# LemonATsu/DANBO-pytorch

Measured on AMD Instinct MI355X. Metric: ray-samples/sec at 512x512x64 samples, higher is better.
Workload: dtype f32 (fp16x2-split MFMA products, fp32 accumulate); 1 GPU; H36M danbo_base network, 512x512 rays x (48 coarse + 16 importance) samples, 1 pose / 1 camera per rank, cylinder near/far, exact in-volume culling; rays=262144, samples_per_ray=64, parallelism=rays-dp1

## Files before the change

danbo-pytorch_amd/core/render_engine.py:

```python
import ctypes

import torch

from . import _hip
from . import hip_ops as ops


class RenderEngine:
    fuse_resample = False

    def _key(self):
        return tuple((k, v.data_ptr(), v._version) for k, v in sorted(self.p.items()))

    def _sampling(self, N_samples, N_importance):
        cfg = self.cfg
        return (N_samples or cfg["N_samples"], N_importance or cfg["N_importance"], cfg["density_scale"],
                ops.density_act(cfg.get("density_act")))

    @staticmethod
    def frame_result(out, out0):
        return dict(rgb_map=out["rgb_map"], disp_map=out["disp_map"], acc_map=out["acc_map"], alpha=out["alpha"],
                    T_i=out["weights"], rgb0=out0["rgb_map"], disp0=out0["disp_map"], acc0=out0["acc_map"],
                    alpha0=out0["alpha"])

# ... 20 lines not shown
        ret = self.frame_result(out, out0)
        if keep:
            ret.update(near=near, far=far, z_coarse=z, raw_coarse=raw, weights_coarse=out0["weights"], z_fine=z_fine,
                       z_sorted=z_all, sorted_idxs=order, raw_fine=raw_f, **ex, **ex_f)
        return ret


class DanboEngine(RenderEngine):
    fuse_resample = True

    def __init__(self, cfg, params, align, buffers=None, mlp_mode="f16split"):
        self.cfg = cfg
        self.p = params
        self.align = align.float().contiguous()
        self._packed_key = None
        self.packed = self.wrt = self.empty_consts = None
        self.mean_code = None
        self.profile = None
        self.skip_flat_rays = True
        self.mlp_form = 32
        assert mlp_mode in ("f16split", "fp32")
        self.mlp_mode = mlp_mode
        self.group_rows = False

    def refresh(self):
        key = self._key()
        if key == self._packed_key and getattr(self, "_built_mode", None) == (self.mlp_mode, self.mlp_form):
            return
        p = self.p
        dev = p["alpha_linear.weight"].device
        q = self._equalized(p) if self.mlp_mode == "f16split" else p
        self.pts_w = [q[f"pts_linears.{i}.weight"] for i in range(8)]
        self.pts_b = [q[f"pts_linears.{i}.bias"].contiguous() for i in range(8)]
        self.packed, self.wrt = ops.mlp_pack(self.pts_w, q["feature_linear.weight"], q["views_linears.0.weight"])
        self.packed16, self.views_b16 = ops.mlp16_pack(self.pts_w, q["feature_linear.weight"],
                                                       q["feature_linear.bias"], q["views_linears.0.weight"],
                                                       q["views_linears.0.bias"], form=self.mlp_form)
        self.alpha_w = q["alpha_linear.weight"].reshape(-1).contiguous()
        self.alpha_b = q["alpha_linear.bias"].contiguous()
        self.feature_b = q["feature_linear.bias"].contiguous()
        self.views_b = q["views_linears.0.bias"].contiguous()
        self.rgb_w = q["rgb_linear.weight"].contiguous()
        self.rgb_b = q["rgb_linear.bias"].contiguous()
        self.view_scale = q.get("_view_scale", torch.ones((), device=dev))
        g = "graph_net.layers."
        self.gw = dict(
# ... 198 lines not shown
        o = _hip.DanboFrameOut(**{k: v.data_ptr() for k, v in out.items()})
        nbytes = _hip.lib().danbo_render_frame_workspace(R, G, S, Sf, int(chunk), m.graph_width)
        ws = torch.empty(nbytes, device=dev, dtype=torch.uint8)
        ops._call("danbo_render_frame_act", ctypes.byref(m), ctypes.byref(r), S, Sf, ctypes.byref(o), _hip.ptr(ws), nbytes,
                  *ops._act_args(act), ops._stream())
        out["T_i"] = out.pop("weights")
        return out

    def near_far(self, rays_o, rays_d, cyls, skts, near0=0.0, far0=1.0, chunk=4096):
        self.refresh()
        near, far = ops.near_far_cylinder(rays_o, rays_d, cyls, near0, far0, chunk)
        if self.cfg["use_volume_near_far"]:
            ops.near_far_boxes(rays_o, rays_d, skts, self.align, self.axis_scale, near, far)
        return near, far

    def render(self, rays_o, rays_d, skts, bones, cyls, cam_idx=None, N_samples=None, N_importance=None,
               chunk=4096, near_far=None, dense=False, keep=False):
        S, Sf, B, act = self._sampling(N_samples, N_importance)
        self.refresh()
        fused = S <= 64 and Sf <= 64
        lazy = not dense and not keep
        flat_mode = (lazy and (fused or (S <= 256 and Sf <= 64)) and self.skip_flat_rays and self.flat_rays_ok
                     and act[0] == "relu")
        near, far = self.near_far(rays_o, rays_d, cyls, skts, 0.0, 1.0, chunk) if near_far is None else near_far
        z = ops.coarse_samples(near, far, S)
        ray_mask = None if dense else ops.ray_bone_mask(rays_o, rays_d, skts, self.align, self.axis_scale, near, far,
                                                        want_flat=flat_mode)
        counts = torch.zeros(3, device=rays_o.device, dtype=torch.int32)
        flat = None
        vols = self.volumes(bones)
        if flat_mode:
            flat = ops.flat_rays(ray_mask[1], ray_mask[3], S, Sf, want_weights=not fused, cnt=counts[2:3])
            view = self.view_constants(rays_d, skts, cam_idx, flat["ray_list"], flat["ray_count"])
        else:
            view = self.view_constants(rays_d, skts, cam_idx)
        if ray_mask is not None:
            ray_mask = ray_mask[:3]
        raw, ex = self.forward_samples(rays_o, rays_d, skts, bones, cam_idx, z=z, dense=dense, volumes=vols, view=view,
                                       fill=not lazy, ray_mask=ray_mask, count=counts[0:1])
        if fused:
            out0, z_all, z_fine, order = ops.composite_importance(
                raw, z, rays_d, Sf, B, bits=ex["valid_bits"] if lazy else None, raw_empty=view[1] if lazy else None,
                want_weights=keep, flat=flat, act=act)
        else:
            out0 = ops.composite(raw, z, rays_d, B, bits=ex["valid_bits"] if lazy else None, raw_empty=view[1] if lazy else None,
                                 flat=flat, act=act)
# ... 22 lines not shown
```

danbo-pytorch_amd/csrc/k_frame.hip:

```cpp
#include "common.hpp"

using namespace danbo;

namespace {
struct Carver {
    char* base;
    size_t used, cap;
    template <class T>
    T* take(size_t n) {
        used = (used + 255) & ~(size_t)255;
        T* p = base ? reinterpret_cast<T*>(base + used) : nullptr;
        used += n * sizeof(T);
        return p;
    }
};

struct FrameBuffers {
    float *near, *far, *cyl_scratch, *z, *vol_scratch, *volumes, *cview, *raw_empty, *h, *raw_a, *raw_b, *z_fine, *z_sorted, *weights0;
    uint32_t *bits_a, *bits_b, *ray_mask, *ray_flat;
    int32_t *list, *count, *order, *ray_list;
};

FrameBuffers carve(Carver& c, int R, int G, int S, int Sf, int chunk, int Wg) {
    FrameBuffers b;
    const size_t M = (size_t)R * S, Mf = (size_t)R * Sf;
    b.near = c.take<float>(R);
    b.far = c.take<float>(R);
    b.cyl_scratch = c.take<float>(8 * (size_t)((R + chunk - 1) / chunk));
    b.z = c.take<float>(M);
    b.vol_scratch = c.take<float>(3 * (size_t)G * 24 * Wg);
    b.volumes = c.take<float>((size_t)G * 24 * 240);
    b.cview = c.take<float>((size_t)R * 128);
    b.raw_empty = c.take<float>((size_t)R * 4);
    b.ray_mask = c.take<uint32_t>(R);
    b.ray_flat = c.take<uint32_t>(R);
    b.ray_list = c.take<int32_t>(R);
    b.bits_a = c.take<uint32_t>(M);
    b.bits_b = c.take<uint32_t>(Mf);
    b.list = c.take<int32_t>(M);
    b.count = c.take<int32_t>(4);
    b.h = c.take<float>((M > Mf ? M : Mf) * 16);
    b.raw_a = c.take<float>(M * 4);
    b.raw_b = c.take<float>(Mf * 4);
    b.z_fine = c.take<float>(Mf);
    b.z_sorted = c.take<float>(M + Mf);
    b.order = c.take<int32_t>(M + Mf);
    if (Mf > M) b.list = c.take<int32_t>(Mf);
    b.weights0 = (S <= 64 && Sf <= 64) ? nullptr : c.take<float>(M);
    return b;
}
}

extern "C" size_t danbo_render_frame_workspace(int R, int G, int S, int Sf, int chunk, int graph_width) {
    if (R < 1 || G < 1 || S < 1 || Sf < 1 || chunk < 1 || graph_width < 1) return 0;
    Carver c{nullptr, 0, 0};
    carve(c, R, G, S, Sf, chunk, graph_width);
    return c.used + 256;
}

#define DANBO_TRY(call) do { const int rc_ = (call); if (rc_ != 0) return rc_; } while (0)

static int render_frame_impl(const DanboModel* m, const DanboRays* r, int S, int Sf, const DanboFrameOut* o, void* workspace,
                             size_t workspace_bytes, int act, float shift, void* stream) {
    DANBO_CHECK_ARG(m && r && o && workspace && S >= 3 && S <= 256 && Sf >= 1 && Sf <= 64);
    DANBO_CHECK_ARG(r->R >= 1 && r->G >= 1 && r->R % r->G == 0 && r->chunk >= 1);
    DANBO_CHECK_ARG(r->rays_o && r->rays_d && r->skts && r->bones && r->cyls);
    DANBO_CHECK_ARG(o->rgb_map && o->disp_map && o->acc_map && o->alpha && o->weights && o->rgb0 && o->disp0 && o->acc0 && o->alpha0);
    const int R = r->R, G = r->G;
    const bool flat_rays = m->flat_rays_ok != 0 && act == DANBO_DENSITY_RELU;
    DANBO_CHECK_ARG(workspace_bytes >= danbo_render_frame_workspace(R, G, S, Sf, r->chunk, m->graph_width));
    Carver c{reinterpret_cast<char*>(((uintptr_t)workspace + 255) & ~(uintptr_t)255), 0, workspace_bytes};
    const FrameBuffers b = carve(c, R, G, S, Sf, r->chunk, m->graph_width);
    hipStream_t st = (hipStream_t)stream;

    DANBO_TRY(danbo_near_far_cylinder(r->rays_o, r->rays_d, r->cyls, R, G, 0.f, 1.f, r->near_in, r->far_in, r->chunk, b.cyl_scratch,
                                      b.near, b.far, stream));
    if (m->use_volume_near_far)
        DANBO_TRY(danbo_near_far_boxes(r->rays_o, r->rays_d, r->skts, m->align, m->axis_scale, R, G, b.near, b.far, stream));
    DANBO_TRY(danbo_coarse_samples(b.near, b.far, R, S, nullptr, b.z, stream));
    DANBO_TRY(danbo_ray_bone_mask(r->rays_o, r->rays_d, b.near, b.far, R, G, r->skts, m->align, m->axis_scale, b.ray_mask,
                                  flat_rays ? b.ray_flat : nullptr, stream));
    DANBO_TRY(danbo_pose_volumes_fwd(r->bones, G, m->L_graph, m->graph_width, m->g_w0, m->g_adjw0, m->g_b0, m->g_w1, m->g_adjw1, m->g_b1,
                                     m->g_w2, m->g_b2, m->g_w3, m->g_b3, b.vol_scratch, b.volumes, stream));
    zero_words(b.count, 4, nullptr, 0, st);
    auto view_consts = [&](const int32_t* ray_list, const int32_t* ray_count) -> int {
        return danbo_view_consts(r->rays_d, r->skts, R, G, m->ray_mode, m->normalise, m->L_view, m->framecodes, m->n_codes, m->code_size,
                                 m->mean_code, r->cam_idx, m->views_w_ray_t, m->views_b_eff, m->rgb_w, m->rgb_b, m->empty_consts, 2,
                                 m->code_table, ray_list, ray_count, b.cview, b.raw_empty, stream);
    };
    const int32_t *ray_list = nullptr, *ray_count = nullptr;
    if (flat_rays) {
        DANBO_TRY(danbo_flat_rays(b.near, b.ray_flat, R, S, Sf, o->rgb0, o->disp0, o->acc0, b.weights0, o->alpha0, b.z_fine, o->rgb_map,
                                  o->disp_map, o->acc_map, o->weights, o->alpha, b.ray_list, b.count + 3, 3, stream));
        ray_list = b.ray_list;
        ray_count = b.count + 3;
    }
    DANBO_TRY(view_consts(ray_list, ray_count));
    auto cull = [&](const float* zz, int s, uint32_t* bits, int32_t* count) -> int {
        DANBO_TRY(danbo_bone_cull(r->rays_o, r->rays_d, zz, nullptr, R, s, G, r->skts, m->align, m->axis_scale, b.ray_mask, b.near, b.far,
                                  nullptr, bits, b.list, count, stream));
        return 0;
    };
    auto network = [&](const float* zz, int s, uint32_t* bits, int32_t* count, float* raw) -> int {
        DANBO_TRY(danbo_gather_assign_blend16_fwd(r->rays_o, r->rays_d, zz, nullptr, R, s, G, r->skts, m->align, m->axis_scale, b.volumes,
                                                  bits, b.list, count, R * s, m->assign16, m->a_b0, m->a_b1, m->a_w2, m->a_b2, b.h,
                                                  nullptr, reinterpret_cast<uint32_t*>(b.count + 2), stream));
        return danbo_pe_mlp32_fwd(b.h, b.list, count, R * s, s, m->mlp16, m->pts_b, m->alpha_w, m->alpha_b, b.cview, m->rgb_w,
                                  m->rgb_b, raw, nullptr, stream);
    };
    DANBO_TRY(cull(b.z, S, b.bits_a, b.count));
    DANBO_TRY(network(b.z, S, b.bits_a, b.count, b.raw_a));
    if (S <= 64) {
        DANBO_TRY(danbo_composite_importance_pdf_fwd_act(b.raw_a, b.raw_empty, b.bits_a, b.z, r->rays_d, R, S, Sf, m->density_scale, nullptr,
                                                         nullptr, 0, o->rgb0, o->disp0, o->acc0, nullptr, o->alpha0, b.z_fine, b.z_sorted,
                                                         b.order, ray_list, ray_count, act, shift, stream));
    } else {
        DANBO_TRY(danbo_composite_rays_fwd_act(b.raw_a, b.raw_empty, b.bits_a, b.z, r->rays_d, R, S, m->density_scale, nullptr, o->rgb0,
                                               o->disp0, o->acc0, b.weights0, o->alpha0, ray_list, ray_count, act, shift, stream));
        DANBO_TRY(danbo_importance_samples_rays(b.z, b.weights0, R, S, Sf, nullptr, b.z_fine, b.z_sorted, b.order, ray_list, ray_count,
                                                stream));
    }
    DANBO_TRY(cull(b.z_fine, Sf, b.bits_b, b.count + 1));
    DANBO_TRY(network(b.z_fine, Sf, b.bits_b, b.count + 1, b.raw_b));
// ... 16 lines not shown
```

danbo-pytorch_amd/csrc/k_sample.hip:

```cpp
#include "common.hpp"

namespace danbo {

__global__ __launch_bounds__(256) DANBO_NO_PK_F32 void k_cylinder_pass1(const float* __restrict__ rays_o,
                                                        const float* __restrict__ rays_d,
                                                        const float* __restrict__ cyl, int R, int G,
                                                        float near0, float far0,
                                                        const float* __restrict__ near_in,
                                                        const float* __restrict__ far_in, int chunk,
                                                        double* __restrict__ acc,
                                                        float* __restrict__ near_out,
                                                        float* __restrict__ far_out) {
    const int rays_per_pose = R / G;
    for (int r0 = blockIdx.x * blockDim.x; r0 < R; r0 += gridDim.x * blockDim.x) {
        const int r = r0 + threadIdx.x;
        const bool act = r < R;
        const int rc = act ? r : R - 1;
        const int g = min(rc / rays_per_pose, G - 1);
        float o[3] = {rays_o[3 * rc], rays_o[3 * rc + 1], rays_o[3 * rc + 2]};
        float d[3] = {rays_d[3 * rc], rays_d[3 * rc + 1], rays_d[3 * rc + 2]};
        float c[3] = {cyl[5 * g], cyl[5 * g + 1], cyl[5 * g + 2]};
        float nr, fr;
        const bool hit = cylinder_bounds(o, d, c, near_in ? near_in[rc] : near0, far_in ? far_in[rc] : far0, &nr, &fr) && act;
        if (act) {
// ... 241 lines not shown
    bone_local(sk, al, o, ol);
    for (int k = 0; k < 3; ++k) t[k] = sk[4 * k] * d[0] + sk[4 * k + 1] * d[1] + sk[4 * k + 2] * d[2];
    for (int k = 0; k < 3; ++k) dl[k] = al[4 * k] * t[0] + al[4 * k + 1] * t[1] + al[4 * k + 2] * t[2];
    const float pad = 1e-4f * fmaxf(fabsf(zl), fabsf(zh)) + 1e-5f;
    float tmin = zl - pad, tmax = zh + pad;
    bool miss = false;
    for (int k = 0; k < 3; ++k) {
        const float s = sc[k] * 1.001f + 1e-4f;
        if (fabsf(dl[k]) < 1e-12f) {
            miss = miss || fabsf(ol[k]) > s;
        } else {
            const float inv = 1.0f / dl[k];
            const float t1 = (-s - ol[k]) * inv, t2 = (s - ol[k]) * inv;
            tmin = fmaxf(tmin, fminf(t1, t2));
            tmax = fminf(tmax, fmaxf(t1, t2));
        }
    }
    return miss || tmin > tmax;
}

constexpr float RAY_FLAT_VMAX = DANBO_RAY_FLAT_VMAX;

template <bool POSES_IN_LDS>
__global__ __launch_bounds__(256) void k_ray_bone_mask(const float* __restrict__ rays_o, const float* __restrict__ rays_d,
                                                       const float* __restrict__ t_lo, const float* __restrict__ t_hi,
                                                       const float* __restrict__ skts, const float* __restrict__ align,
                                                       const float* __restrict__ axis_scale, int R, int G,
                                                       uint32_t* __restrict__ ray_mask, uint32_t* __restrict__ ray_flat) {
    extern __shared__ __attribute__((aligned(16))) float smem[];
    float* s_align = smem;
    float* s_scale = smem + J * 16;
    float* s_skt = smem + J * 16 + J * 4;
    const int rays_per_pose = R / G;
    const int r_a = blockIdx.x * 256, r_b = min(r_a + 255, R - 1);
    const int g0 = min(r_a / rays_per_pose, G - 1), g1 = min(r_b / rays_per_pose, G - 1);
    const int r = min(r_a + (int)threadIdx.x, R - 1);
    const float o[3] = {rays_o[3 * r], rays_o[3 * r + 1], rays_o[3 * r + 2]};
    const float d[3] = {rays_d[3 * r], rays_d[3 * r + 1], rays_d[3 * r + 2]};
    const float zl = t_lo[r], zh = t_hi[r];
    for (int i = threadIdx.x; i < J * 16; i += 256) s_align[i] = align[i];
    for (int i = threadIdx.x; i < J * 4; i += 256) s_scale[i] = (i & 3) < 3 ? fabsf(axis_scale[(i >> 2) * 3 + (i & 3)]) : 0.f;
    if (POSES_IN_LDS)
        for (int i = threadIdx.x; i < (g1 - g0 + 1) * J * 16; i += 256) s_skt[i] = skts[(size_t)g0 * J * 16 + i];
    __syncthreads();
    const int g = min(r / rays_per_pose, G - 1);
    uint32_t bits = 0u;
    if (POSES_IN_LDS) {
        const float* sk = s_skt + (size_t)(g - g0) * J * 16;
#pragma unroll 2
        for (int j = 0; j < J; ++j)
            bits |= segment_misses_bone(sk + 16 * j, s_align + 16 * j, s_scale + 4 * j, o, d, zl, zh) ? 0u : 1u << j;
    } else {
        for (int j = 0; j < J; ++j) {
            float sk[12];
            const float* src = skts + ((size_t)g * J + j) * 16;
#pragma unroll
            for (int i = 0; i < 12; ++i) sk[i] = src[i];
            bits |= segment_misses_bone(sk, s_align + 16 * j, s_scale + 4 * j, o, d, zl, zh) ? 0u : 1u << j;
        }
    }
    if (r_a + (int)threadIdx.x < R) {
        ray_mask[r] = bits;
        if (ray_flat != nullptr) {
            const float dn = norm3_torch(d[0], d[1], d[2]);
            const float span = mul_rn(add_rn(sub_rn(zh, zl), mul_rn(1e-3f, fmaxf(fabsf(zl), fabsf(zh)))), dn);
            const float tail = mul_rn(1e10f, dn);
            const float* m0 = POSES_IN_LDS ? s_skt + (size_t)(g - g0) * J * 16 : skts + (size_t)g * J * 16;
            float msum = 0.f;
            for (int a = 0; a < 3; ++a)
                for (int k = 0; k < 3; ++k) msum = add_rn(msum, fabsf(m0[4 * a + k]));
            const float vin = mul_rn(dn, fmaxf(1.0f, msum));
            const bool fin = zl <= zh && sub_rn(span, span) == 0.f && sub_rn(tail, tail) == 0.f && vin <= RAY_FLAT_VMAX;
            ray_flat[r] = (bits == 0u && fin) ? 1u : 0u;
        }
    }
}

constexpr int CULL_BLOCK = 256;
constexpr int CULL_SPT = 4;
constexpr int CULL_MAX_RAYS = 130;

__global__ __launch_bounds__(CULL_BLOCK) void k_bone_cull(const float* __restrict__ rays_o,
                                                          const float* __restrict__ rays_d,
                                                          const float* __restrict__ z,
                                                          const float* __restrict__ pts, int R, int S, int G,
                                                          const float* __restrict__ skts,
                                                          const float* __restrict__ align,
                                                          const float* __restrict__ axis_scale, int np_lds,
                                                          const uint32_t* __restrict__ ray_mask,
                                                          const float* __restrict__ t_lo, const float* __restrict__ t_hi,
                                                          uint32_t* __restrict__ ray_flat,
                                                          uint32_t* __restrict__ valid_bits,
                                                          int32_t* __restrict__ list, int32_t* __restrict__ count) {
    extern __shared__ __attribute__((aligned(16))) float smem[];
    float* s_align = smem;
    float* s_scale = smem + J * 16;
    float* s_skt = smem + J * 16 + J * 4;
    __shared__ float s_zlo[CULL_MAX_RAYS], s_zhi[CULL_MAX_RAYS];
    __shared__ uint32_t s_mask[CULL_MAX_RAYS];

    const long M = (long)R * S;
    const long spp = (long)(R / G) * S;
    const long base = (long)blockIdx.x * (CULL_BLOCK * CULL_SPT);
// ... 92 lines not shown
        const int lia = (int)(mac - base) + off0, lib = (int)(mbc - base) + off0;
        const int ra = r_first + ray_of(lia), rb = r_first + ray_of(lib);
        float pa[3], pb[3];
        if (pts != nullptr) {
            pa[0] = pts[3 * mac]; pa[1] = pts[3 * mac + 1]; pa[2] = pts[3 * mac + 2];
            pb[0] = pts[3 * mbc]; pb[1] = pts[3 * mbc + 1]; pb[2] = pts[3 * mbc + 2];
        } else {
            const float oa[3] = {rays_o[3 * ra], rays_o[3 * ra + 1], rays_o[3 * ra + 2]};
            const float da[3] = {rays_d[3 * ra], rays_d[3 * ra + 1], rays_d[3 * ra + 2]};
            const float ob[3] = {rays_o[3 * rb], rays_o[3 * rb + 1], rays_o[3 * rb + 2]};
            const float db[3] = {rays_d[3 * rb], rays_d[3 * rb + 1], rays_d[3 * rb + 2]};
            sample_point(oa, da, ma < M ? zreg[2 * pr] : z[M - 1], pa);
            sample_point(ob, db, mb < M ? zreg[2 * pr + 1] : z[M - 1], pb);
        }
        const int ga = pose_of(ra), gb = pose_of(rb);
        uint32_t ba = 0, bb = 0;
        uint32_t need = (1u << J) - 1u;
        if (ray_mask != nullptr) {
            need = wave_or(pre[2 * pr] | pre[2 * pr + 1]);
        } else if (prefilter) {
            uint32_t mine = s_mask[ra - r_first] | s_mask[rb - r_first];
            need = wave_or(mine);
        }
        if (__builtin_amdgcn_readfirstlane((int)__all(ga == gb))) {
            const v2f px = {pa[0], pb[0]}, py = {pa[1], pb[1]}, pz = {pa[2], pb[2]};
            const float* sk = s_skt + (ga - g0) * J * 16;
            while (need) {
                const int j = __builtin_ctz(need);
                need &= need - 1u;
                v2f l[3], t[3];
                affine_pk(sk + 16 * j, px, py, pz, l);
                affine_pk(s_align + 16 * j, l[0], l[1], l[2], t);
                const float* sc = s_scale + 4 * j;
                const bool ina = !(fabsf(t[0].x) > sc[0] || fabsf(t[1].x) > sc[1] || fabsf(t[2].x) > sc[2]);
                const bool inb = !(fabsf(t[0].y) > sc[0] || fabsf(t[1].y) > sc[1] || fabsf(t[2].y) > sc[2]);
                ba |= (ina ? 1u : 0u) << j;
                bb |= (inb ? 1u : 0u) << j;
            }
        } else {
            const float* ska = s_skt + (ga - g0) * J * 16;
            const float* skb = s_skt + (gb - g0) * J * 16;
            for (int j = 0; j < J; ++j) {
                float pt[3];
                bone_local(ska + 16 * j, s_align + 16 * j, pa, pt);
                ba |= (in_volume(pt, s_scale + 4 * j) ? 1u : 0u) << j;
                bone_local(skb + 16 * j, s_align + 16 * j, pb, pt);
                bb |= (in_volume(pt, s_scale + 4 * j) ? 1u : 0u) << j;
            }
        }
        bits4[2 * pr] = ma < M ? ba : 0u;
        bits4[2 * pr + 1] = mb < M ? bb : 0u;
        if (ma < M) valid_bits[ma] = ba;
        if (mb < M) valid_bits[mb] = bb;
    }
    if (list != nullptr) {
        __shared__ int s_cnt[CULL_SPT * (CULL_BLOCK / 64)];
        __shared__ int s_base;
        const int wave = threadIdx.x >> 6;
        unsigned long long ball[CULL_SPT];
#pragma unroll
        for (int it = 0; it < CULL_SPT; ++it) {
            ball[it] = __ballot(bits4[it] != 0);
            if (lane == 0) s_cnt[it * (CULL_BLOCK / 64) + wave] = __popcll(ball[it]);
        }
        __syncthreads();
        if (threadIdx.x == 0) {
            int run = 0;
            for (int i = 0; i < CULL_SPT * (CULL_BLOCK / 64); ++i) { const int c = s_cnt[i]; s_cnt[i] = run; run += c; }
            s_base = run > 0 ? atomicAdd(count, run) : 0;
        }
        __syncthreads();
#pragma unroll
        for (int it = 0; it < CULL_SPT; ++it) {
            if (bits4[it] != 0) {
                const long m = base + it * CULL_BLOCK + threadIdx.x;
                list[s_base + s_cnt[it * (CULL_BLOCK / 64) + wave] + __popcll(ball[it] & ((1ull << lane) - 1ull))] = (int32_t)m;
            }
        }
    }
}

constexpr int GATHER_TS = 16;
constexpr int GATHER_BLOCK = GATHER_TS * J;

__global__ __launch_bounds__(GATHER_BLOCK) void k_bone_gather(const float* __restrict__ rays_o,
                                                              const float* __restrict__ rays_d,
                                                              const float* __restrict__ z,
                                                              const float* __restrict__ pts, int R, int S, int G,
                                                              const float* __restrict__ skts,
                                                              const float* __restrict__ align,
                                                              const float* __restrict__ axis_scale,
                                                              const float* __restrict__ volumes,
                                                              const int32_t* __restrict__ list,
                                                              const int32_t* __restrict__ count, int n_cap,
                                                              float* __restrict__ part_feat) {
    __shared__ __attribute__((aligned(16))) float s_vol[J * VOL];
    __shared__ __attribute__((aligned(16))) float s_out[GATHER_TS * J * FEAT];
    __shared__ __attribute__((aligned(16))) float s_skt[J * 16];
    __shared__ __attribute__((aligned(16))) float s_align[J * 16];
    __shared__ float s_scale[J * 4];

    const int n = resolve_count(count, n_cap);
// ... 528 lines not shown
        for (int c = lane; c < S; c += 64) {
            if (weights0) weights0[rr * S + c] = 0.f;
            if (alpha0) alpha0[rr * S + c] = 0.f;
        }
        const float lo_b = __builtin_bit_cast(float, __builtin_amdgcn_readlane(__builtin_bit_cast(int, lo), b));
        for (int c = lane; c < Sf; c += 64) z_fine[rr * Sf + c] = lo_b;
        for (int c = lane; c < St; c += 64) {
            if (weights) weights[rr * St + c] = 0.f;
            if (alpha_out) alpha_out[rr * St + c] = 0.f;
        }
    }
    if (!(parts & 1)) return;
    if (lane == 0) s_cnt[wave] = (int)__popcll(listed);
    __syncthreads();
    if (threadIdx.x == 0) {
        int run = 0;
        for (int w = 0; w < FLAT_BLOCK / 64; ++w) { const int c = s_cnt[w]; s_cnt[w] = run; run += c; }
        s_base = run > 0 ? atomicAdd(ray_count, run) : 0;
    }
    __syncthreads();
    if (r < R && !flat) ray_list[s_base + s_cnt[wave] + (int)__popcll(listed & ((1ull << lane) - 1ull))] = r;
}

}

using namespace danbo;

static unsigned ray_scatter(int R) {
    static const unsigned primes[] = {40507u, 40519u, 40529u, 40531u, 40543u, 40559u};
    for (unsigned p : primes) {
        unsigned a = p, b = (unsigned)R;
        while (b != 0u) { const unsigned t = a % b; a = b; b = t; }
        if (a == 1u) return p;
    }
    return 1u;
}

extern "C" int danbo_near_far_cylinder(const float* rays_o, const float* rays_d, const float* cyl, int R, int G,
                                        float near0, float far0, const float* near_in, const float* far_in, int chunk,
                                        float* scratch, float* near_out, float* far_out, void* stream) {
    DANBO_CHECK_ARG(R > 0 && G > 0 && R % G == 0 && chunk > 0 && scratch != nullptr);
    hipStream_t st = (hipStream_t)stream;
    const int nchunk = ceil_div(R, chunk);
    if (chunk <= CYL_FUSED_MAX) {
        hipLaunchKernelGGL(k_cylinder_chunk, dim3(nchunk), dim3(CYL_BLOCK), 0, st, rays_o, rays_d, cyl, R, G, near0, far0, near_in,
                           far_in, chunk, near_out, far_out);
// ... 28 lines not shown
                           far, R, S, t_rand, z);
    DANBO_LAUNCH_RET();
}

extern "C" int danbo_bone_cull(const float* rays_o, const float* rays_d, const float* z, const float* pts, int R, int S, int G,
                                const float* skts, const float* align, const float* axis_scale, const uint32_t* ray_mask,
                                const float* t_lo, const float* t_hi, uint32_t* ray_flat, uint32_t* valid_bits, int32_t* list,
                                int32_t* count, void* stream) {
    DANBO_CHECK_ARG(R > 0 && S > 0 && G > 0 && R % G == 0);
    DANBO_CHECK_ARG((list == nullptr) == (count == nullptr));
    DANBO_CHECK_ARG((z == nullptr) != (pts == nullptr));
    DANBO_CHECK_ARG(ray_mask == nullptr || (z != nullptr && t_lo != nullptr && t_hi != nullptr));
    DANBO_CHECK_ARG(ray_flat == nullptr || ray_mask != nullptr);
    const long M = (long)R * S;
    const long spp = (long)(R / G) * S;
    const int per_block = CULL_BLOCK * CULL_SPT;
    long np = per_block / spp + 2;
    if (np > G) np = G;
    const size_t lds = sizeof(float) * (J * 16 + J * 4 + np * J * 16);
    DANBO_CHECK_ARG(lds <= 64 * 1024);
    const int grid = ceil_div(M, per_block);
    hipLaunchKernelGGL(k_bone_cull, dim3(grid), dim3(CULL_BLOCK), lds, (hipStream_t)stream, rays_o, rays_d, z, pts, R, S,
                       G, skts, align, axis_scale, (int)np, ray_mask, t_lo, t_hi, ray_flat, valid_bits, list, count);
    DANBO_LAUNCH_RET();
}

extern "C" int danbo_ray_bone_mask(const float* rays_o, const float* rays_d, const float* t_lo, const float* t_hi, int R, int G,
                                    const float* skts, const float* align, const float* axis_scale, uint32_t* ray_mask,
                                    uint32_t* ray_flat, void* stream) {
    DANBO_CHECK_ARG(rays_o && rays_d && t_lo && t_hi && skts && align && axis_scale && ray_mask);
    DANBO_CHECK_ARG(R > 0 && G > 0 && R % G == 0);
    const long np = 256 / (R / G) + 2 < G ? 256 / (R / G) + 2 : G;
    const bool in_lds = np <= 8;
    const size_t lds = sizeof(float) * (J * 16 + J * 4 + (in_lds ? np * J * 16 : 0));
    if (in_lds)
        hipLaunchKernelGGL(k_ray_bone_mask<true>, dim3(ceil_div(R, 256)), dim3(256), lds, (hipStream_t)stream, rays_o, rays_d, t_lo, t_hi,
                           skts, align, axis_scale, R, G, ray_mask, ray_flat);
    else
        hipLaunchKernelGGL(k_ray_bone_mask<false>, dim3(ceil_div(R, 256)), dim3(256), lds, (hipStream_t)stream, rays_o, rays_d, t_lo,
                           t_hi, skts, align, axis_scale, R, G, ray_mask, ray_flat);
    DANBO_LAUNCH_RET();
}

extern "C" int danbo_bone_gather_fwd(const float* rays_o, const float* rays_d, const float* z, const float* pts, int R, int S, int G,
                                      const float* skts, const float* align, const float* axis_scale,
                                      const float* volumes, const int32_t* list, const int32_t* count, int n,
// ... 157 lines not shown
                                                       int act, float shift, void* stream) {
    DANBO_CHECK_ARG(pdf == 0 || pdf == 1);
    DANBO_CHECK_DENSITY_ACT(act, shift);
#define DANBO_CI(TWO_, DA_, SH_)                                                                                                   \
    composite_importance_impl<TWO_, DA_>(raw, raw_empty, valid_bits, z, rays_d, R, S, Sf, B, noise, u, rgb_map, disp, acc, weights, \
                                         alpha, z_fine, z_sorted, sorted_idx, ray_list, ray_count, SH_, stream)
    if (act == DENSITY_SOFTPLUS) return pdf ? DANBO_CI(true, DENSITY_SOFTPLUS, shift) : DANBO_CI(false, DENSITY_SOFTPLUS, shift);
    return pdf ? DANBO_CI(true, DENSITY_RELU, 0.f) : DANBO_CI(false, DENSITY_RELU, 0.f);
#undef DANBO_CI
}

extern "C" int danbo_flat_rays(const float* t_lo, const uint32_t* ray_flat, int R, int S, int Sf, float* rgb0, float* disp0, float* acc0, float* weights0, float* alpha0, float* z_fine,
                                float* rgb_map, float* disp, float* acc, float* weights, float* alpha, int32_t* ray_list,
                                int32_t* ray_count, int parts, void* stream) {
    DANBO_CHECK_ARG(R > 0 && S >= 3 && Sf > 0);
    DANBO_CHECK_ARG(t_lo && ray_flat && rgb0 && disp0 && acc0 && z_fine && rgb_map && disp && acc && ray_list && ray_count);
    DANBO_CHECK_ARG(parts >= 1 && parts <= 3);
    hipLaunchKernelGGL(k_flat_rays, dim3(ceil_div(R, FLAT_BLOCK)), dim3(FLAT_BLOCK), 0, (hipStream_t)stream,
                       t_lo, ray_flat, R, S, Sf, rgb0, disp0, acc0, weights0, alpha0, z_fine,
                       rgb_map, disp, acc, weights, alpha, ray_list, ray_count, parts);
    DANBO_LAUNCH_RET();
}

template <int DA>
static int composite_merged_impl(const float* raw_a, const float* raw_b, const float* raw_empty,
                                 const uint32_t* bits_a, const uint32_t* bits_b, const int32_t* sorted_idx,
                                 const float* z_sorted, const float* rays_d, int R, int S, int Sf, float B,
                                 const float* noise, float* rgb_map, float* disp, float* acc, float* weights,
                                 float* alpha, float* raw_sorted, const int32_t* ray_list, const int32_t* ray_count,
                                 float shift, void* stream) {
    DANBO_CHECK_ARG(R > 0 && S > 0 && Sf > 0 && B > 0.f && raw_a && raw_b && sorted_idx && z_sorted && rays_d);
    DANBO_CHECK_ARG(rgb_map && disp && acc && ((bits_a == nullptr && bits_b == nullptr) || raw_empty != nullptr));
    DANBO_CHECK_ARG((ray_list == nullptr) == (ray_count == nullptr));
    const float4 *a4 = reinterpret_cast<const float4*>(raw_a), *b4 = reinterpret_cast<const float4*>(raw_b);
    const float4* e4 = reinterpret_cast<const float4*>(raw_empty);
    float4* rs4 = reinterpret_cast<float4*>(raw_sorted);
    if constexpr (DA == DENSITY_SOFTPLUS) {
        static const int per_launch = resident_grid(k_composite_merged_softplus, 1L << 40, 256);
        hipLaunchKernelGGL(k_composite_merged_softplus, dim3((unsigned)std::min<long>(ceil_div((long)R * 64, 256), per_launch)), dim3(256), 0,
                           (hipStream_t)stream, a4, b4, e4, bits_a, bits_b, sorted_idx, z_sorted, rays_d, R, S, Sf, B, noise, rgb_map, disp, acc,
                           weights, alpha, rs4, ray_list, ray_count, ray_scatter(R), shift);
    } else {
        static const int per_launch = resident_grid(k_composite_merged, 1L << 40, 256);
        hipLaunchKernelGGL(k_composite_merged, dim3((unsigned)std::min<long>(ceil_div((long)R * 64, 256), per_launch)), dim3(256), 0,
                           (hipStream_t)stream, a4, b4, e4, bits_a, bits_b, sorted_idx, z_sorted, rays_d, R, S, Sf, B, noise, rgb_map, disp, acc,
                           weights, alpha, rs4, ray_list, ray_count, ray_scatter(R));
// ... 27 lines not shown
```

Measured before the change: 3.798 billion ray-samples/s.

## Fuse ray front-end into one kernel and cull only non-flat rays in C frame path

Adds a k_ray_front kernel that merges bone-mask candidate testing, flat-ray output zeroing, compaction of non-flat rays into a list, and coarse z-sample generation, so several kernel launches and intermediate buffers go away. Adds k_bone_cull_rays, which culls samples only for rays in the compacted list instead of all rays. The Python render path now sends eligible flat-mode frames to the single C frame renderer. The cost is more complex indexing (ray_of via float division), a wider LDS footprint, and a dependence on device-side ray_count for the grid.

After: 3.769 billion ray-samples/s. Within noise of the previous version (-0.8%).

```diff
diff --git a/danbo-pytorch_amd/core/render_engine.py b/danbo-pytorch_amd/core/render_engine.py
--- a/danbo-pytorch_amd/core/render_engine.py
+++ b/danbo-pytorch_amd/core/render_engine.py
@@ -66,6 +66,7 @@
         assert mlp_mode in ("f16split", "fp32")
         self.mlp_mode = mlp_mode
         self.group_rows = False
+        self.frame_in_c = True
 
     def refresh(self):
         key = self._key()
@@ -310,6 +311,9 @@
         lazy = not dense and not keep
         flat_mode = (lazy and (fused or (S <= 256 and Sf <= 64)) and self.skip_flat_rays and self.flat_rays_ok
                      and act[0] == "relu")
+        if (flat_mode and self.frame_in_c and near_far is None and self.mlp_form == 32 and not self.group_rows
+                and self.profile is None):
+            return self.render_frame_c(rays_o, rays_d, skts, bones, cyls, cam_idx, S, Sf, chunk)
         near, far = self.near_far(rays_o, rays_d, cyls, skts, 0.0, 1.0, chunk) if near_far is None else near_far
         z = ops.coarse_samples(near, far, S)
         ray_mask = None if dense else ops.ray_bone_mask(rays_o, rays_d, skts, self.align, self.axis_scale, near, far,
diff --git a/danbo-pytorch_amd/csrc/k_frame.hip b/danbo-pytorch_amd/csrc/k_frame.hip
--- a/danbo-pytorch_amd/csrc/k_frame.hip
+++ b/danbo-pytorch_amd/csrc/k_frame.hip
@@ -1,4 +1,5 @@
 #include "common.hpp"
+#include "ray_chain.hpp"
 
 using namespace danbo;
 
@@ -17,7 +18,7 @@
 
 struct FrameBuffers {
     float *near, *far, *cyl_scratch, *z, *vol_scratch, *volumes, *cview, *raw_empty, *h, *raw_a, *raw_b, *z_fine, *z_sorted, *weights0;
-    uint32_t *bits_a, *bits_b, *ray_mask, *ray_flat;
+    uint32_t *bits_a, *bits_b, *ray_mask;
     int32_t *list, *count, *order, *ray_list;
 };
 
@@ -33,7 +34,6 @@
     b.cview = c.take<float>((size_t)R * 128);
     b.raw_empty = c.take<float>((size_t)R * 4);
     b.ray_mask = c.take<uint32_t>(R);
-    b.ray_flat = c.take<uint32_t>(R);
     b.ray_list = c.take<int32_t>(R);
     b.bits_a = c.take<uint32_t>(M);
     b.bits_b = c.take<uint32_t>(Mf);
@@ -77,28 +77,34 @@
                                       b.near, b.far, stream));
     if (m->use_volume_near_far)
         DANBO_TRY(danbo_near_far_boxes(r->rays_o, r->rays_d, r->skts, m->align, m->axis_scale, R, G, b.near, b.far, stream));
-    DANBO_TRY(danbo_coarse_samples(b.near, b.far, R, S, nullptr, b.z, stream));
-    DANBO_TRY(danbo_ray_bone_mask(r->rays_o, r->rays_d, b.near, b.far, R, G, r->skts, m->align, m->axis_scale, b.ray_mask,
-                                  flat_rays ? b.ray_flat : nullptr, stream));
+    zero_words(b.count, 4, nullptr, 0, st);
+    const int32_t *ray_list = nullptr, *ray_count = nullptr;
+    if (flat_rays) {
+        DANBO_TRY(danbo_ray_front(r->rays_o, r->rays_d, b.near, b.far, R, G, S, Sf, r->skts, m->align, m->axis_scale, b.ray_mask, nullptr, b.z,
+                                  o->rgb0, o->disp0, o->acc0, b.weights0, o->alpha0, o->rgb_map, o->disp_map, o->acc_map, o->weights, o->alpha,
+                                  b.ray_list, b.count + 3, stream));
+        ray_list = b.ray_list;
+        ray_count = b.count + 3;
+    } else {
+        DANBO_TRY(danbo_coarse_samples(b.near, b.far, R, S, nullptr, b.z, stream));
+        DANBO_TRY(danbo_ray_bone_mask(r->rays_o, r->rays_d, b.near, b.far, R, G, r->skts, m->align, m->axis_scale, b.ray_mask, nullptr,
+                                      stream));
+    }
     DANBO_TRY(danbo_pose_volumes_fwd(r->bones, G, m->L_graph, m->graph_width, m->g_w0, m->g_adjw0, m->g_b0, m->g_w1, m->g_adjw1, m->g_b1,
                                      m->g_w2, m->g_b2, m->g_w3, m->g_b3, b.vol_scratch, b.volumes, stream));
-    zero_words(b.count, 4, nullptr, 0, st);
     auto view_consts = [&](const int32_t* ray_list, const int32_t* ray_count) -> int {
         return danbo_view_consts(r->rays_d, r->skts, R, G, m->ray_mode, m->normalise, m->L_view, m->framecodes, m->n_codes, m->code_size,
                                  m->mean_code, r->cam_idx, m->views_w_ray_t, m->views_b_eff, m->rgb_w, m->rgb_b, m->empty_consts, 2,
                                  m->code_table, ray_list, ray_count, b.cview, b.raw_empty, stream);
     };
-    const int32_t *ray_list = nullptr, *ray_count = nullptr;
-    if (flat_rays) {
-        DANBO_TRY(danbo_flat_rays(b.near, b.ray_flat, R, S, Sf, o->rgb0, o->disp0, o->acc0, b.weights0, o->alpha0, b.z_fine, o->rgb_map,
-                                  o->disp_map, o->acc_map, o->weights, o->alpha, b.ray_list, b.count + 3, 3, stream));
-        ray_list = b.ray_list;
-        ray_count = b.count + 3;
-    }
     DANBO_TRY(view_consts(ray_list, ray_count));
     auto cull = [&](const float* zz, int s, uint32_t* bits, int32_t* count) -> int {
-        DANBO_TRY(danbo_bone_cull(r->rays_o, r->rays_d, zz, nullptr, R, s, G, r->skts, m->align, m->axis_scale, b.ray_mask, b.near, b.far,
-                                  nullptr, bits, b.list, count, stream));
+        if (flat_rays)
+            DANBO_TRY(danbo_bone_cull_rays(r->rays_o, r->rays_d, zz, R, s, G, r->skts, m->align, m->axis_scale, b.ray_mask, b.near, b.far,
+                                           ray_list, ray_count, bits, b.list, count, 0, stream));
+        else
+            DANBO_TRY(danbo_bone_cull(r->rays_o, r->rays_d, zz, nullptr, R, s, G, r->skts, m->align, m->axis_scale, b.ray_mask, b.near,
+                                      b.far, nullptr, bits, b.list, count, stream));
         return 0;
     };
     auto network = [&](const float* zz, int s, uint32_t* bits, int32_t* count, float* raw) -> int {
diff --git a/danbo-pytorch_amd/csrc/k_sample.hip b/danbo-pytorch_amd/csrc/k_sample.hip
--- a/danbo-pytorch_amd/csrc/k_sample.hip
+++ b/danbo-pytorch_amd/csrc/k_sample.hip
@@ -1,4 +1,5 @@
 #include "common.hpp"
+#include "ray_chain.hpp"
 
 namespace danbo {
 
@@ -287,12 +288,11 @@
 constexpr float RAY_FLAT_VMAX = DANBO_RAY_FLAT_VMAX;
 
 template <bool POSES_IN_LDS>
-__global__ __launch_bounds__(256) void k_ray_bone_mask(const float* __restrict__ rays_o, const float* __restrict__ rays_d,
-                                                       const float* __restrict__ t_lo, const float* __restrict__ t_hi,
-                                                       const float* __restrict__ skts, const float* __restrict__ align,
-                                                       const float* __restrict__ axis_scale, int R, int G,
-                                                       uint32_t* __restrict__ ray_mask, uint32_t* __restrict__ ray_flat) {
-    extern __shared__ __attribute__((aligned(16))) float smem[];
+__device__ __forceinline__ uint32_t ray_candidates(const float* __restrict__ rays_o, const float* __restrict__ rays_d,
+                                                   const float* __restrict__ t_lo, const float* __restrict__ t_hi,
+                                                   const float* __restrict__ skts, const float* __restrict__ align,
+                                                   const float* __restrict__ axis_scale, int R, int G, float* smem, bool want_flat,
+                                                   float& zl, float& zh, bool& flat) {
     float* s_align = smem;
     float* s_scale = smem + J * 16;
     float* s_skt = smem + J * 16 + J * 4;
@@ -302,7 +302,8 @@
     const int r = min(r_a + (int)threadIdx.x, R - 1);
     const float o[3] = {rays_o[3 * r], rays_o[3 * r + 1], rays_o[3 * r + 2]};
     const float d[3] = {rays_d[3 * r], rays_d[3 * r + 1], rays_d[3 * r + 2]};
-    const float zl = t_lo[r], zh = t_hi[r];
+    zl = t_lo[r];
+    zh = t_hi[r];
     for (int i = threadIdx.x; i < J * 16; i += 256) s_align[i] = align[i];
     for (int i = threadIdx.x; i < J * 4; i += 256) s_scale[i] = (i & 3) < 3 ? fabsf(axis_scale[(i >> 2) * 3 + (i & 3)]) : 0.f;
     if (POSES_IN_LDS)
@@ -324,26 +325,71 @@
             bits |= segment_misses_bone(sk, s_align + 16 * j, s_scale + 4 * j, o, d, zl, zh) ? 0u : 1u << j;
         }
     }
-    if (r_a + (int)threadIdx.x < R) {
+    flat = false;
+    if (want_flat) {
+        const float dn = norm3_torch(d[0], d[1], d[2]);
+        const float span = mul_rn(add_rn(sub_rn(zh, zl), mul_rn(1e-3f, fmaxf(fabsf(zl), fabsf(zh)))), dn);
+        const float tail = mul_rn(1e10f, dn);
+        const float* m0 = POSES_IN_LDS ? s_skt + (size_t)(g - g0) * J * 16 : skts + (size_t)g * J * 16;
+        float msum = 0.f;
+        for (int a = 0; a < 3; ++a)
+            for (int k = 0; k < 3; ++k) msum = add_rn(msum, fabsf(m0[4 * a + k]));
+        const float vin = mul_rn(dn, fmaxf(1.0f, msum));
+        const bool fin = zl <= zh && sub_rn(span, span) == 0.f && sub_rn(tail, tail) == 0.f && vin <= RAY_FLAT_VMAX;
+        flat = bits == 0u && fin;
+    }
+    return bits;
+}
+
+template <bool POSES_IN_LDS>
+__global__ __launch_bounds__(256) void k_ray_bone_mask(const float* __restrict__ rays_o, const float* __restrict__ rays_d,
+                                                       const float* __restrict__ t_lo, const float* __restrict__ t_hi,
+                                                       const float* __restrict__ skts, const float* __restrict__ align,
+                                                       const float* __restrict__ axis_scale, int R, int G,
+                                                       uint32_t* __restrict__ ray_mask, uint32_t* __restrict__ ray_flat) {
+    extern __shared__ __attribute__((aligned(16))) float smem[];
+    float zl, zh;
+    bool flat;
+    const uint32_t bits = ray_candidates<POSES_IN_LDS>(rays_o, rays_d, t_lo, t_hi, skts, align, axis_scale, R, G, smem, ray_flat != nullptr,
+                                                       zl, zh, flat);
+    const int r = blockIdx.x * 256 + (int)threadIdx.x;
+    if (r < R) {
         ray_mask[r] = bits;
-        if (ray_flat != nullptr) {
-            const float dn = norm3_torch(d[0], d[1], d[2]);
-            const float span = mul_rn(add_rn(sub_rn(zh, zl), mul_rn(1e-3f, fmaxf(fabsf(zl), fabsf(zh)))), dn);
-            const float tail = mul_rn(1e10f, dn);
-            const float* m0 = POSES_IN_LDS ? s_skt + (size_t)(g - g0) * J * 16 : skts + (size_t)g * J * 16;
-            float msum = 0.f;
-            for (int a = 0; a < 3; ++a)
-                for (int k = 0; k < 3; ++k) msum = add_rn(msum, fabsf(m0[4 * a + k]));
-            const float vin = mul_rn(dn, fmaxf(1.0f, msum));
-            const bool fin = zl <= zh && sub_rn(span, span) == 0.f && sub_rn(tail, tail) == 0.f && vin <= RAY_FLAT_VMAX;
-            ray_flat[r] = (bits == 0u && fin) ? 1u : 0u;
-        }
+        if (ray_flat != nullptr) ray_flat[r] = flat ? 1u : 0u;
     }
 }
 
 constexpr int CULL_BLOCK = 256;
 constexpr int CULL_SPT = 4;
 constexpr int CULL_MAX_RAYS = 130;
+
+__device__ __forceinline__ void cull_pair(const float* pa, const float* pb, const float* sk, const float* ska, const float* skb,
+                                          bool packed, uint32_t need, const float* s_align, const float* s_scale, uint32_t& ba,
+                                          uint32_t& bb) {
+    if (packed) {
+        const v2f px = {pa[0], pb[0]}, py = {pa[1], pb[1]}, pz = {pa[2], pb[2]};
+        while (need) {
+            const int j = __builtin_ctz(need);
+            need &= need - 1u;
+            v2f l[3], t[3];
+            affine_pk(sk + 16 * j, px, py, pz, l);
+            affine_pk(s_align + 16 * j, l[0], l[1], l[2], t);
+            const float* sc = s_scale + 4 * j;
+            const bool ina = !(fabsf(t[0].x) > sc[0] || fabsf(t[1].x) > sc[1] || fabsf(t[2].x) > sc[2]);
+            const bool inb = !(fabsf(t[0].y) > sc[0] || fabsf(t[1].y) > sc[1] || fabsf(t[2].y) > sc[2]);
+            ba |= (ina ? 1u : 0u) << j;
+            bb |= (inb ? 1u : 0u) << j;
+        }
+    } else {
+        for (int j = 0; j < J; ++j) {
+            float pt[3];
+            bone_local(ska + 16 * j, s_align + 16 * j, pa, pt);
+            ba |= (in_volume(pt, s_scale + 4 * j) ? 1u : 0u) << j;
+            bone_local(skb + 16 * j, s_align + 16 * j, pb, pt);
+            bb |= (in_volume(pt, s_scale + 4 * j) ? 1u : 0u) << j;
+        }
+    }
+}
 
 __global__ __launch_bounds__(CULL_BLOCK) void k_bone_cull(const float* __restrict__ rays_o,
                                                           const float* __restrict__ rays_d,
@@ -482,32 +528,8 @@
             uint32_t mine = s_mask[ra - r_first] | s_mask[rb - r_first];
             need = wave_or(mine);
         }
-        if (__builtin_amdgcn_readfirstlane((int)__all(ga == gb))) {
-            const v2f px = {pa[0], pb[0]}, py = {pa[1], pb[1]}, pz = {pa[2], pb[2]};
-            const float* sk = s_skt + (ga - g0) * J * 16;
-            while (need) {
-                const int j = __builtin_ctz(need);
-                need &= need - 1u;
-                v2f l[3], t[3];
-                affine_pk(sk + 16 * j, px, py, pz, l);
-                affine_pk(s_align + 16 * j, l[0], l[1], l[2], t);
-                const float* sc = s_scale + 4 * j;
-                const bool ina = !(fabsf(t[0].x) > sc[0] || fabsf(t[1].x) > sc[1] || fabsf(t[2].x) > sc[2]);
-                const bool inb = !(fabsf(t[0].y) > sc[0] || fabsf(t[1].y) > sc[1] || fabsf(t[2].y) > sc[2]);
-                ba |= (ina ? 1u : 0u) << j;
-                bb |= (inb ? 1u : 0u) << j;
-            }
-        } else {
-            const float* ska = s_skt + (ga - g0) * J * 16;
-            const float* skb = s_skt + (gb - g0) * J * 16;
-            for (int j = 0; j < J; ++j) {
-                float pt[3];
-                bone_local(ska + 16 * j, s_align + 16 * j, pa, pt);
-                ba |= (in_volume(pt, s_scale + 4 * j) ? 1u : 0u) << j;
-                bone_local(skb + 16 * j, s_align + 16 * j, pb, pt);
-                bb |= (in_volume(pt, s_scale + 4 * j) ? 1u : 0u) << j;
-            }
-        }
+        cull_pair(pa, pb, s_skt + (ga - g0) * J * 16, s_skt + (ga - g0) * J * 16, s_skt + (gb - g0) * J * 16,
+                  __builtin_amdgcn_readfirstlane((int)__all(ga == gb)) != 0, need, s_align, s_scale, ba, bb);
         bits4[2 * pr] = ma < M ? ba : 0u;
         bits4[2 * pr + 1] = mb < M ? bb : 0u;
         if (ma < M) valid_bits[ma] = ba;
@@ -538,6 +560,167 @@
             }
         }
     }
+}
+
+constexpr int CULL_WINDOW = CULL_BLOCK * CULL_SPT;
+constexpr int CULL_RAYS_MAX_POSES = 8;
+constexpr int CULL_MAX_WINDOWS = 4;
+
+__global__ __launch_bounds__(CULL_BLOCK) void k_bone_cull_rays(const float* __restrict__ rays_o, const float* __restrict__ rays_d,
+                                                               const float* __restrict__ z, int R, int S, int G, int W,
+                                                               const float* __restrict__ skts, const float* __restrict__ align,
+                                                               const float* __restrict__ axis_scale, int np_lds,
+                                                               const uint32_t* __restrict__ ray_mask, const float* __restrict__ t_lo,
+                                                               const float* __restrict__ t_hi, const int32_t* __restrict__ ray_list,
+                                                               const int32_t* __restrict__ ray_count, uint32_t* __restrict__ valid_bits,
+                                                               int32_t* __restrict__ list, int32_t* __restrict__ count) {
+    extern __shared__ __attribute__((aligned(16))) float smem[];
+    float* s_align = smem;
+    float* s_scale = smem + J * 16;
+    float* s_skt = smem + J * 16 + J * 4;
+    int* s_ray = reinterpret_cast<int*>(s_skt + np_lds * J * 16);
+    __shared__ int s_g0;
+    constexpr int NC = CULL_MAX_WINDOWS * CULL_SPT * (CULL_BLOCK / 64);
+    static_assert(NC <= 64, "one wavefront scans the group counts");
+    __shared__ int s_cnt[NC];
+    __shared__ unsigned long long s_ball[NC];
+
+    const int n = min(max(*ray_count, 0), R);
+    const long M = (long)n * S;
+    const long base0 = (long)blockIdx.x * (W * CULL_WINDOW);
+    if (base0 >= M) return;
+    const long last = min(base0 + W * CULL_WINDOW, M) - 1;
+    const int lane = threadIdx.x & 63, wave = threadIdx.x >> 6;
+    const int i_first = (int)(base0 / S), i_last = (int)(last / S);
+    const int off0 = (int)(base0 - (long)i_first * S);
+    const int nrays = i_last - i_first + 1;
+    const int rays_per_pose = R / G;
+    const float inv_S = 1.0f / (float)S;
+    auto ray_of = [&](int li) {
+        int q = (int)((float)li * inv_S);
+        q -= (q * S > li) ? 1 : 0;
+        q += ((q + 1) * S <= li) ? 1 : 0;
+        return q;
+    };
+    auto pose_of = [&](int r) { return G == 1 ? 0 : min(r / rays_per_pose, G - 1); };
+    const int nitems = (int)(last - base0) + 1;
+    auto item = [&](int w, int k) { return w * CULL_WINDOW + k * CULL_BLOCK + (int)threadIdx.x; };
+    auto sample_of = [&](int it, unsigned& r) {
+        const int li = min(it, nitems - 1) + off0;
+        const int q = ray_of(li);
+        r = (unsigned)s_ray[q];
+        return r * (unsigned)S + (unsigned)(li - q * S);
+    };
+
+    if (threadIdx.x == 0) s_g0 = G - 1;
+    int gmin = G - 1;
+    for (int i = threadIdx.x; i < nrays; i += CULL_BLOCK) {
+        const int r = min(max(ray_list[i_first + i], 0), R - 1);
+        s_ray[i] = r;
+        gmin = min(gmin, pose_of(r));
+    }
+    for (int i = threadIdx.x; i < J * 16; i += CULL_BLOCK) s_align[i] = align[i];
+    for (int i = threadIdx.x; i < J * 4; i += CULL_BLOCK) s_scale[i] = (i & 3) < 3 ? fabsf(axis_scale[(i >> 2) * 3 + (i & 3)]) : 0.f;
+    __syncthreads();
+    if (gmin < G - 1) atomicMin(&s_g0, gmin);
+    __syncthreads();
+    const int g0 = s_g0;
+    const int npose = min(np_lds, G - g0);
+    for (int i = threadIdx.x; i < npose * J * 16; i += CULL_BLOCK) s_skt[i] = skts[(size_t)g0 * J * 16 + i];
+    __syncthreads();
+
+    for (int i = threadIdx.x; i < NC; i += CULL_BLOCK) { s_cnt[i] = 0; s_ball[i] = 0ull; }
+    __syncthreads();
+#pragma unroll 1
+    for (int w = 0; w < W && w * CULL_WINDOW < nitems; ++w) {
+        float zreg[CULL_SPT];
+        uint32_t pre[CULL_SPT];
+        bool any = false;
+#pragma unroll
+        for (int k = 0; k < CULL_SPT; ++k) {
+            unsigned r;
+            zreg[k] = z[sample_of(item(w, k), r)];
+            const float lo = t_lo[r], hi = t_hi[r];
+            const float slack = 5e-5f * fmaxf(fabsf(lo), fabsf(hi));
+            const bool inside = zreg[k] >= lo - slack && zreg[k] <= hi + slack;
+            pre[k] = item(w, k) >= nitems ? 0u : inside ? ray_mask[r] : (1u << J) - 1u;
+            any = any || pre[k] != 0u;
+        }
+        if (!__syncthreads_or(any ? 1 : 0)) {
+#pragma unroll
+            for (int k = 0; k < CULL_SPT; ++k)
+                if (item(w, k) < nitems) { unsigned r; valid_bits[sample_of(item(w, k), r)] = 0u; }
+            continue;
+        }
+#pragma unroll
+        for (int pr = 0; pr < CULL_SPT / 2; ++pr) {
+            const int a = 2 * pr, b = 2 * pr + 1;
+            unsigned ra, rb;
+            const unsigned ma = sample_of(item(w, a), ra), mb = sample_of(item(w, b), rb);
+            const float oa[3] = {rays_o[3 * ra], rays_o[3 * ra + 1], rays_o[3 * ra + 2]};
+            const float da[3] = {rays_d[3 * ra], rays_d[3 * ra + 1], rays_d[3 * ra + 2]};
+            const float ob[3] = {rays_o[3 * rb], rays_o[3 * rb + 1], rays_o[3 * rb + 2]};
+            const float db[3] = {rays_d[3 * rb], rays_d[3 * rb + 1], rays_d[3 * rb + 2]};
+            float pa[3], pb[3];
+            sample_point(oa, da, zreg[a], pa);
+            sample_point(ob, db, zreg[b], pb);
+            const int ga = pose_of((int)ra) - g0, gb = pose_of((int)rb) - g0;
+            const bool packed = __builtin_amdgcn_readfirstlane((int)__all(ga == gb && ga < npose)) != 0;
+            uint32_t ba = 0, bb = 0;
+            if (packed) {
+                const float* sk = s_skt + ga * J * 16;
+                cull_pair(pa, pb, sk, sk, sk, true, wave_or(pre[a] | pre[b]), s_align, s_scale, ba, bb);
+            } else {
+                const float* ska = skts + (size_t)(ga + g0) * J * 16;
+                const float* skb = skts + (size_t)(gb + g0) * J * 16;
+#pragma unroll 1
+                for (int j = 0; j < J; ++j) {
+                    float pt[3];
+                    bone_local(ska + 16 * j, s_align + 16 * j, pa, pt);
+                    ba |= (in_volume(pt, s_scale + 4 * j) ? 1u : 0u) << j;
+                    bone_local(skb + 16 * j, s_align + 16 * j, pb, pt);
+                    bb |= (in_volume(pt, s_scale + 4 * j) ? 1u : 0u) << j;
+                }
+            }
+            if (item(w, a) >= nitems) ba = 0u;
+            else valid_bits[ma] = ba;
+            if (item(w, b) >= nitems) bb = 0u;
+            else valid_bits[mb] = bb;
+            const unsigned long long balla = __ballot(ba != 0u), ballb = __ballot(bb != 0u);
+            if (lane == 0) {
+                const int ia = (w * CULL_SPT + a) * (CULL_BLOCK / 64) + wave, ib = ia + CULL_BLOCK / 64;
+                s_ball[ia] = balla; s_cnt[ia] = __popcll(balla);
+                s_ball[ib] = ballb; s_cnt[ib] = __popcll(ballb);
+            }
+        }
+    }
+    __syncthreads();
+    if (wave == 0) {
+        const int c = s_cnt[lane];
+        int inc = c;
+#pragma unroll
+        for (int off = 1; off < 64; off <<= 1) {
+            const int t = __shfl_up(inc, off, 64);
+            if (lane >= off) inc += t;
+        }
+        const int total = __shfl(inc, 63, 64);
+        int first = 0;
+        if (lane == 0 && total > 0) first = atomicAdd(count, total);
+        first = __shfl(first, 0, 64);
+        s_cnt[lane] = first + inc - c;
+    }
+    __syncthreads();
+#pragma unroll 1
+    for (int w = 0; w < W && w * CULL_WINDOW < nitems; ++w)
+#pragma unroll
+        for (int k = 0; k < CULL_SPT; ++k) {
+            const int i = (w * CULL_SPT + k) * (CULL_BLOCK / 64) + wave;
+            const unsigned long long ball = s_ball[i];
+            if ((ball >> lane) & 1ull) {
+                unsigned r;
+                list[s_cnt[i] + __popcll(ball & ((1ull << lane) - 1ull))] = (int32_t)sample_of(item(w, k), r);
+            }
+        }
 }
 
 constexpr int GATHER_TS = 16;
@@ -1112,6 +1295,80 @@
     if (r < R && !flat) ray_list[s_base + s_cnt[wave] + (int)__popcll(listed & ((1ull << lane) - 1ull))] = r;
 }
 
+template <class F>
+__device__ __forceinline__ void wave_rows(float* __restrict__ base, int n, size_t r0, unsigned long long owners, int lane, F value) {
+    if (base == nullptr || owners == 0ull) return;
+    float* rows = base + r0 * n;
+    const float inv_n = 1.0f / (float)n;
+    for (int idx = lane; idx < 64 * n; idx += 64) {
+        int b = (int)((float)idx * inv_n);
+        b -= (b * n > idx) ? 1 : 0;
+        b += ((b + 1) * n <= idx) ? 1 : 0;
+        const float v = value(b, idx - b * n);
+        if ((owners >> b) & 1ull) rows[idx] = v;
+    }
+}
+__device__ __forceinline__ void wave_zero_rows(float* __restrict__ base, int n, size_t r0, unsigned long long owners, int lane) {
+    if (base != nullptr && owners == ~0ull && (reinterpret_cast<uintptr_t>(base) & 15) == 0) {
+        float4* rows = reinterpret_cast<float4*>(base + r0 * n);
+        for (int i = lane; i < 16 * n; i += 64) rows[i] = float4{0.f, 0.f, 0.f, 0.f};
+        return;
+    }
+    wave_rows(base, n, r0, owners, lane, [](int, int) { return 0.f; });
+}
+
+template <bool POSES_IN_LDS>
+__global__ __launch_bounds__(256) void k_ray_front(const float* __restrict__ rays_o, const float* __restrict__ rays_d,
+                                                   const float* __restrict__ t_lo, const float* __restrict__ t_hi,
+                                                   const float* __restrict__ skts, const float* __restrict__ align,
+                                                   const float* __restrict__ axis_scale, int R, int G, int S, int Sf,
+                                                   uint32_t* __restrict__ ray_mask, uint32_t* __restrict__ ray_flat, float* __restrict__ z,
+                                                   float* __restrict__ rgb0, float* __restrict__ disp0, float* __restrict__ acc0,
+                                                   float* __restrict__ weights0, float* __restrict__ alpha0,
+                                                   float* __restrict__ rgb_map, float* __restrict__ disp, float* __restrict__ acc_out,
+                                                   float* __restrict__ weights, float* __restrict__ alpha_out,
+                                                   int32_t* __restrict__ ray_list, int32_t* __restrict__ ray_count) {
+    extern __shared__ __attribute__((aligned(16))) float smem[];
+    __shared__ int s_cnt[256 / 64];
+    __shared__ int s_base;
+    const int lane = threadIdx.x & 63, wave = threadIdx.x >> 6;
+    float zl, zh;
+    bool fl;
+    const uint32_t bits = ray_candidates<POSES_IN_LDS>(rays_o, rays_d, t_lo, t_hi, skts, align, axis_scale, R, G, smem, true, zl, zh, fl);
+    const int r = blockIdx.x * 256 + (int)threadIdx.x;
+    const bool flat = r < R && fl, other = r < R && !fl;
+    if (r < R) {
+        ray_mask[r] = bits;
+        if (ray_flat != nullptr) ray_flat[r] = fl ? 1u : 0u;
+    }
+    if (flat) {
+        rgb0[3 * r] = 0.f; rgb0[3 * r + 1] = 0.f; rgb0[3 * r + 2] = 0.f;
+        disp0[r] = 0.f;
+        acc0[r] = 0.f;
+        rgb_map[3 * r] = 0.f; rgb_map[3 * r + 1] = 0.f; rgb_map[3 * r + 2] = 0.f;
+        disp[r] = 0.f;
+        acc_out[r] = 0.f;
+    }
+    const unsigned long long flats = __ballot(flat), listed = __ballot(other);
+    if (lane == 0) s_cnt[wave] = (int)__popcll(listed);
+    __syncthreads();
+    if (threadIdx.x == 0) {
+        int run = 0;
+        for (int w = 0; w < 256 / 64; ++w) { const int c = s_cnt[w]; s_cnt[w] = run; run += c; }
+        s_base = run > 0 ? atomicAdd(ray_count, run) : 0;
+    }
+    __syncthreads();
+    if (other) ray_list[s_base + s_cnt[wave] + (int)__popcll(listed & ((1ull << lane) - 1ull))] = r;
+    const size_t r0 = (size_t)blockIdx.x * 256 + wave * 64;
+    wave_rows(z, S, r0, listed, lane, [&](int b, int s) {
+        return coarse_sample(__shfl(zl, b, 64), __shfl(zh, b, 64), s, S, nullptr, 0);
+    });
+    wave_zero_rows(weights0, S, r0, flats, lane);
+    wave_zero_rows(alpha0, S, r0, flats, lane);
+    wave_zero_rows(weights, S + Sf, r0, flats, lane);
+    wave_zero_rows(alpha_out, S + Sf, r0, flats, lane);
+}
+
 }
 
 using namespace danbo;
@@ -1186,6 +1443,23 @@
     const int grid = ceil_div(M, per_block);
     hipLaunchKernelGGL(k_bone_cull, dim3(grid), dim3(CULL_BLOCK), lds, (hipStream_t)stream, rays_o, rays_d, z, pts, R, S,
                        G, skts, align, axis_scale, (int)np, ray_mask, t_lo, t_hi, ray_flat, valid_bits, list, count);
+    DANBO_LAUNCH_RET();
+}
+
+extern "C" int danbo_bone_cull_rays(const float* rays_o, const float* rays_d, const float* z, int R, int S, int G, const float* skts,
+                                     const float* align, const float* axis_scale, const uint32_t* ray_mask, const float* t_lo,
+                                     const float* t_hi, const int32_t* ray_list, const int32_t* ray_count, uint32_t* valid_bits,
+                                     int32_t* list, int32_t* count, int windows, void* stream) {
+    DANBO_CHECK_ARG(R > 0 && S > 0 && G > 0 && R % G == 0 && (long)R * S <= 0x7fffffffL);
+    DANBO_CHECK_ARG(rays_o && rays_d && z && skts && align && axis_scale && ray_mask && t_lo && t_hi && ray_list && ray_count);
+    DANBO_CHECK_ARG(valid_bits && list && count);
+    DANBO_CHECK_ARG(windows >= 0 && windows <= CULL_MAX_WINDOWS);
+    if (windows == 0) windows = (long)R * S >= 8L * CULL_MAX_WINDOWS * CULL_WINDOW * num_cu() ? CULL_MAX_WINDOWS : 1;
+    const int np = G < CULL_RAYS_MAX_POSES ? G : CULL_RAYS_MAX_POSES;
+    const size_t lds = sizeof(float) * (J * 16 + J * 4 + np * J * 16 + windows * CULL_WINDOW / S + 2);
+    hipLaunchKernelGGL(k_bone_cull_rays, dim3(ceil_div((long)R * S, windows * CULL_WINDOW)), dim3(CULL_BLOCK), lds, (hipStream_t)stream,
+                       rays_o, rays_d, z, R, S, G, windows, skts, align, axis_scale, np, ray_mask, t_lo, t_hi, ray_list, ray_count,
+                       valid_bits, list, count);
     DANBO_LAUNCH_RET();
 }
 
@@ -1389,6 +1663,27 @@
     DANBO_LAUNCH_RET();
 }
 
+extern "C" int danbo_ray_front(const float* rays_o, const float* rays_d, const float* t_lo, const float* t_hi, int R, int G, int S, int Sf,
+                                const float* skts, const float* align, const float* axis_scale, uint32_t* ray_mask, uint32_t* ray_flat,
+                                float* z, float* rgb0, float* disp0, float* acc0, float* weights0, float* alpha0, float* rgb_map,
+                                float* disp, float* acc, float* weights, float* alpha, int32_t* ray_list, int32_t* ray_count,
+                                void* stream) {
+    DANBO_CHECK_ARG(rays_o && rays_d && t_lo && t_hi && skts && align && axis_scale && ray_mask && z);
+    DANBO_CHECK_ARG(rgb0 && disp0 && acc0 && rgb_map && disp && acc && ray_list && ray_count);
+    DANBO_CHECK_ARG(R > 0 && G > 0 && R % G == 0 && S >= 3 && Sf > 0 && S + Sf <= 0x10000);
+    const long np = 256 / (R / G) + 2 < G ? 256 / (R / G) + 2 : G;
+    const bool in_lds = np <= 8;
+    const size_t lds = sizeof(float) * (J * 16 + J * 4 + (in_lds ? np * J * 16 : 0));
+#define DANBO_RAY_FRONT(LDS_)                                                                                                          \
+    hipLaunchKernelGGL(k_ray_front<LDS_>, dim3(ceil_div(R, 256)), dim3(256), lds, (hipStream_t)stream, rays_o, rays_d, t_lo, t_hi, skts, \
+                       align, axis_scale, R, G, S, Sf, ray_mask, ray_flat, z, rgb0, disp0, acc0, weights0, alpha0, rgb_map, disp, acc,  \
+                       weights, alpha, ray_list, ray_count)
+    if (in_lds) DANBO_RAY_FRONT(true);
+    else DANBO_RAY_FRONT(false);
+#undef DANBO_RAY_FRONT
+    DANBO_LAUNCH_RET();
+}
+
 template <int DA>
 static int composite_merged_impl(const float* raw_a, const float* raw_b, const float* raw_empty,
                                  const uint32_t* bits_a, const uint32_t* bits_b, const int32_t* sorted_idx,
diff --git a/danbo-pytorch_amd/csrc/ray_chain.hpp b/danbo-pytorch_amd/csrc/ray_chain.hpp
--- /dev/null
+++ b/danbo-pytorch_amd/csrc/ray_chain.hpp
@@ -0,0 +1,16 @@
+#pragma once
+#include <cstdint>
+
+extern "C" {
+int danbo_bone_cull_rays(const float* rays_o, const float* rays_d, const float* z , int R, int S, int G,
+                         const float* skts , const float* align , const float* axis_scale ,
+                         const uint32_t* ray_mask , const float* t_lo , const float* t_hi ,
+                         const int32_t* ray_list , const int32_t* ray_count , uint32_t* valid_bits ,
+                         int32_t* list , int32_t* count , int windows, void* stream);
+
+int danbo_ray_front(const float* rays_o, const float* rays_d, const float* t_lo , const float* t_hi , int R, int G, int S,
+                    int Sf, const float* skts, const float* align, const float* axis_scale, uint32_t* ray_mask ,
+                    uint32_t* ray_flat , float* z , float* rgb0, float* disp0, float* acc0, float* weights0,
+                    float* alpha0, float* rgb_map, float* disp, float* acc, float* weights , float* alpha,
+                    int32_t* ray_list , int32_t* ray_count , void* stream);
+}
```
